# LiZhuoHong/SegLand

Measured on AMD Instinct MI355X. Metric: 512x512 tiles/sec fwd+bwd PSPNet-POP, higher is better.
Workload: dtype bf16; 1 GPU; PSPNet-POP resnet50 bf16, batch 16/GPU, 512x512, 8 logit channels, train_base.py loop body (fwd+loss+bwd+clip+AdamW x2), 1 x MI355X; global_batch=16, parallelism=dp1

## Files before the change

### include/segland_hip_debug.h

```cpp
#ifndef SEGLAND_HIP_DEBUG_H
#define SEGLAND_HIP_DEBUG_H
#include "segland_hip.h"
#ifdef __cplusplus
extern "C" {
#endif

void sl_debug_reset(void);

void sl_debug_conv_affine(int on);
void sl_debug_conv_p9(int on);
void sl_debug_conv_p9_lean(int on);
void sl_debug_conv_p8_k1(int on);
void sl_debug_conv_ring192(int on);
void sl_debug_conv_ringn64(int on);
void sl_debug_conv_rows_small(int on);
void sl_debug_ppm_fact_walk(int on);
void sl_debug_conv_parity(int on);
void sl_debug_ring_small_k(int k);
void sl_debug_ring64_max_tiles(int tiles);
void sl_debug_wgrad3(int on);
void sl_debug_wgrad_bias(int on);
void sl_debug_wgrad_tr(int on);
void sl_debug_wgrad_pair_min(int rows);
void sl_debug_attn_valu(int v);
void sl_debug_ce_tiled(int on);

void sl_debug_p8_trace(void* buf);
void sl_debug_wgrad_trace(void* buf);
void sl_debug_wgrad3_trace(void* buf);
void sl_debug_attn_trace(void* buf);

int sl_debug_wgrad3_plan(const SlConvDesc* d, int* out);

#ifdef __cplusplus
}
#endif
#endif
```

### segland_amd/csrc/api.cpp

```cpp
#include <stdarg.h>
#include <stdio.h>
#include <mutex>
#include <unordered_map>
#include "common.h"

static thread_local char g_err[512] = "";

void sl_set_error(const char* fmt, ...) {
  va_list ap;
  va_start(ap, fmt);
  vsnprintf(g_err, sizeof(g_err), fmt, ap);
  va_end(ap);
}

extern "C" int sl_version(void) { return 100; }
extern "C" const char* sl_last_error_string(void) { return g_err; }

__attribute__((visibility("hidden"))) int sl_lds_opt_in(const char* name, const void* kernel, size_t lds_bytes) {
  static std::mutex mu;
  static std::unordered_map<const void*, size_t> granted;
  std::lock_guard<std::mutex> lock(mu);
  size_t& have = granted[kernel];
  if (lds_bytes <= have) return 0;
  const hipError_t e = hipFuncSetAttribute(kernel, hipFuncAttributeMaxDynamicSharedMemorySize, (int)lds_bytes);
  if (e != hipSuccess) {
    sl_set_error("%s: opt-in to %zu bytes of dynamic LDS refused: %s", name, lds_bytes, hipGetErrorString(e));
    return (int)e;
  }
  have = lds_bytes;
  return 0;
}

extern "C" int sl_hip_clear_error(void) { return (int)hipGetLastError(); }

#include "../../include/segland_hip_debug.h"
SlDebugState g_sl_debug;
extern "C" void sl_debug_reset(void) { g_sl_debug = SlDebugState(); }
extern "C" void sl_debug_conv_affine(int v) { g_sl_debug.conv_affine = v ? 1 : 0; }
extern "C" void sl_debug_conv_p9(int v) { g_sl_debug.conv_p9 = (v & 1) ? 1 : 0; }
extern "C" void sl_debug_conv_p9_lean(int v) { g_sl_debug.conv_p9_lean = v ? 1 : 0; }
extern "C" void sl_debug_conv_p8_k1(int v) { g_sl_debug.conv_p8_k1 = v ? 1 : 0; }
extern "C" void sl_debug_conv_ring192(int v) { g_sl_debug.conv_ring192 = v ? 1 : 0; }
extern "C" void sl_debug_conv_ringn64(int v) { g_sl_debug.conv_ringn64 = v ? 1 : 0; }
extern "C" void sl_debug_conv_rows_small(int v) { g_sl_debug.conv_rows_small = v ? 1 : 0; }
extern "C" void sl_debug_conv_parity(int v) { g_sl_debug.conv_parity = v ? 1 : 0; }
extern "C" void sl_debug_ppm_fact_walk(int v) { g_sl_debug.ppm_fact_walk = v ? 1 : 0; }
extern "C" void sl_debug_ring64_max_tiles(int v) { g_sl_debug.ring64_max_tiles = v; }
extern "C" void sl_debug_ring_small_k(int v) { g_sl_debug.ring_small_k = v; }
extern "C" void sl_debug_wgrad3(int v) { g_sl_debug.wgrad3 = v ? 1 : 0; }
extern "C" void sl_debug_wgrad_bias(int v) { g_sl_debug.wgrad_bias = v ? 1 : 0; }
extern "C" void sl_debug_wgrad_tr(int v) { g_sl_debug.wgrad_tr = v ? 1 : 0; }
extern "C" void sl_debug_wgrad_pair_min(int rows) { g_sl_debug.wgrad_pair_min_rows = rows; }
extern "C" void sl_debug_attn_valu(int v) { g_sl_debug.attn_valu = v; }
extern "C" void sl_debug_ce_tiled(int v) { g_sl_debug.ce_tiled = v ? 1 : 0; }
extern "C" void sl_debug_p8_trace(void* buf) { g_sl_debug.p8_trace = (unsigned long long*)buf; }
extern "C" void sl_debug_wgrad_trace(void* buf) { g_sl_debug.wgrad_trace = (unsigned long long*)buf; }
extern "C" void sl_debug_wgrad3_trace(void* buf) { g_sl_debug.wgrad3_trace = (unsigned long long*)buf; }
extern "C" void sl_debug_attn_trace(void* buf) { g_sl_debug.attn_trace = (unsigned long long*)buf; }
```

### segland_amd/csrc/common.h

```cpp
#pragma once
#include <hip/hip_runtime.h>
#include <stdint.h>
#include <stdio.h>
#include "../../include/segland_hip.h"

typedef unsigned short bf16_t;

typedef __attribute__((ext_vector_type(8))) __bf16 bf16x8_t;
typedef __attribute__((ext_vector_type(16))) float f32x16_t;
typedef __attribute__((ext_vector_type(4))) float f32x4_t;

__device__ __forceinline__ float bf2f(bf16_t v) { return __uint_as_float(((unsigned)v) << 16); }
__device__ __forceinline__ bf16_t f2bf(float f) {
  return __builtin_bit_cast(bf16_t, (__bf16)f);
}

template <typename T> __device__ __forceinline__ float to_f(T v);
template <> __device__ __forceinline__ float to_f<float>(float v) { return v; }
template <> __device__ __forceinline__ float to_f<bf16_t>(bf16_t v) { return bf2f(v); }
template <typename T> __device__ __forceinline__ T from_f(float v);
template <> __device__ __forceinline__ float from_f<float>(float v) { return v; }
template <> __device__ __forceinline__ bf16_t from_f<bf16_t>(float v) { return f2bf(v); }

template <typename T> struct Vec16 { static constexpr int N = 16 / sizeof(T); };
// ... 6 lines not shown
  out[0] = __uint_as_float(v.x << 16); out[1] = __uint_as_float(v.x & 0xffff0000u);
  out[2] = __uint_as_float(v.y << 16); out[3] = __uint_as_float(v.y & 0xffff0000u);
  out[4] = __uint_as_float(v.z << 16); out[5] = __uint_as_float(v.z & 0xffff0000u);
  out[6] = __uint_as_float(v.w << 16); out[7] = __uint_as_float(v.w & 0xffff0000u);
}
template <typename T> __device__ __forceinline__ uint4 pack16(const float* in);
template <> __device__ __forceinline__ uint4 pack16<float>(const float* in) {
  return make_uint4(__float_as_uint(in[0]), __float_as_uint(in[1]), __float_as_uint(in[2]), __float_as_uint(in[3]));
}
template <> __device__ __forceinline__ uint4 pack16<bf16_t>(const float* in) {
  typedef __attribute__((ext_vector_type(2))) __bf16 bf16x2_t;
  typedef __attribute__((ext_vector_type(2))) float f32x2_t;
  uint4 r;
  r.x = __builtin_bit_cast(unsigned, __builtin_convertvector((f32x2_t){in[0], in[1]}, bf16x2_t));
  r.y = __builtin_bit_cast(unsigned, __builtin_convertvector((f32x2_t){in[2], in[3]}, bf16x2_t));
  r.z = __builtin_bit_cast(unsigned, __builtin_convertvector((f32x2_t){in[4], in[5]}, bf16x2_t));
  r.w = __builtin_bit_cast(unsigned, __builtin_convertvector((f32x2_t){in[6], in[7]}, bf16x2_t));
  return r;
}

__device__ __forceinline__ float sl_erf_as(float x) {
  const float ax = fabsf(x);
  const float t = __builtin_amdgcn_rcpf(fmaf(0.3275911f, ax, 1.f));
  float p = fmaf(1.061405429f, t, -1.453152027f);
  p = fmaf(p, t, 1.421413741f); p = fmaf(p, t, -0.284496736f); p = fmaf(p, t, 0.254829592f);
  const float r = fmaf(-p * t, __expf(-ax * ax), 1.f);
  return copysignf(r, x);
}
template <typename T> __device__ __forceinline__ float sl_gelu(float x) {
  if constexpr (sizeof(T) == 4) return 0.5f * x * (1.f + erff(x * 0.70710678118654752440f));
  else return 0.5f * x * (1.f + sl_erf_as(x * 0.70710678118654752440f));
}

template <typename T> __device__ __forceinline__ float sl_gelu_grad(float x) {
  const float pdf = 0.39894228040143267794f * __expf(-0.5f * x * x);
  float cdf;
  if constexpr (sizeof(T) == 4) cdf = 0.5f * (1.f + erff(x * 0.70710678118654752440f));
  else cdf = 0.5f * (1.f + sl_erf_as(x * 0.70710678118654752440f));
  return cdf + x * pdf;
}

__device__ __forceinline__ float wave_sum(float v) {
#pragma unroll
  for (int o = 32; o > 0; o >>= 1) v += __shfl_xor(v, o, 64);
  return v;
}

void sl_set_error(const char* fmt, ...);

struct SlDebugState {
  int conv_affine = 1;
  int conv_p9 = 1;
  int conv_p9_lean = 1;
  int conv_p8_k1 = 1;
  int conv_ring192 = 1;
  int conv_ringn64 = 1;
  int conv_rows_small = 1;
  int ppm_fact_walk = 1;
  int conv_parity = 1;
  int ring_small_k = 128;
  long long ring64_max_tiles = 256;
  int wgrad3 = 1;
  int wgrad_bias = 1;
  int wgrad_tr = 1;
  long long wgrad_pair_min_rows = 0;
  int attn_valu = -1;
  int ce_tiled = 1;
  unsigned long long* p8_trace = nullptr;
  unsigned long long* wgrad_trace = nullptr;
  unsigned long long* wgrad3_trace = nullptr;
  unsigned long long* attn_trace = nullptr;
};
extern SlDebugState g_sl_debug;
#define SL_REQUIRE(cond, ...)            \
  do {                                   \
    if (!(cond)) {                       \
      sl_set_error(__VA_ARGS__);         \
      return SL_EINVAL;                  \
    }                                    \
  } while (0)
#define SL_TRY(expr)                     \
  do {                                   \
    const int rc__ = (expr);             \
    if (rc__) return rc__;               \
  } while (0)

int sl_lds_opt_in(const char* name, const void* kernel, size_t lds_bytes);

template <typename T> struct sl_as_is { typedef T type; };

template <typename... Args>
static inline int sl_launch(const char* name, void (*kernel)(Args...), dim3 grid, dim3 block, size_t lds_bytes, hipStream_t stream, typename sl_as_is<Args>::type... args) {
  if (lds_bytes > 64 * 1024) SL_TRY(sl_lds_opt_in(name, (const void*)kernel, lds_bytes));
  hipLaunchKernelGGL(kernel, grid, block, lds_bytes, stream, args...);
  const hipError_t e = hipGetLastError();
  if (e != hipSuccess) {
    sl_set_error("%s: %s", name, hipGetErrorString(e));
    return (int)e;
  }
  return 0;
}

template <typename F>
static inline int sl_by_dtype(int dtype, const char* entry, F&& f) {
  if (dtype == SL_BF16) return f(bf16_t());
  if (dtype == SL_F32) return f(float());
// ... 62 lines not shown
```

### segland_amd/csrc/conv_gemm.hip

```cpp
#include "conv_gemm_common.h"

using namespace slconv;
namespace {

constexpr int MIN_TILES256 = 96, RING128_MIN = 16;
static int block_rows(long long M) { return M >= 256LL * MIN_TILES256 ? 256 : 128; }

static int splitk_parts(const ConvGemmParams& p, int dtype) {
  if (dtype != SL_BF16 || p.stat_partial || p.gate || p.mask_src || p.addend_mask || p.out2 || p.row_scale || p.C2 || p.N % 256 || p.M % 256 || p.C1 % 64) return 1;
  const long long tiles = (long long)(p.M / 256) * (p.N / 256);
  if (tiles >= 128 || p.M >= 32768 || p.C1 < 1024) return 1;
  if (!(p9_on() && p.KH == 3 && p.KW == 3 && p.stride == 1 && p.pad == p.dil && (p.dil == 1 || p.dil == 2 || p.dil == 4) && p.Hs == p.Hd && p.Ws == p.Wd && p.Hs % 16 == 0 && p.Ws % 16 == 0))
    return 1;
  const int units = p.C1 / 64;
  int s = 1;
  while (s < 8 && units / (2 * s) >= 4 && tiles * 2 * s <= 256) s *= 2;
  return s;
}

static bool ring192_on() { return g_sl_debug.conv_ring192 != 0; }
static bool rows_small_on() { return g_sl_debug.conv_rows_small != 0; }
static bool ringn64_on() { return g_sl_debug.conv_ringn64 != 0; }

static bool parity_shape(const ConvGemmParams& p) {
// ... 107 lines not shown
  SL_REQUIRE(p.M > 0, "conv: empty output");
  SL_REQUIRE(!(p.gate && p.bias), "conv: no kernel serves a gated data gradient with a bias");
  return launch_gemm(dtype, p, st);
}

int check_desc(const SlConvDesc* d) {
  SL_REQUIRE(d != nullptr, "conv: null descriptor");
  SL_REQUIRE(d->B > 0 && d->H > 0 && d->W > 0 && d->Cin > 0 && d->Cout > 0, "conv: bad sizes");
  SL_REQUIRE(d->KH > 0 && d->KW > 0 && d->stride > 0 && d->dil > 0 && d->pad >= 0, "conv: bad window");
  const int ho = (d->H + 2 * d->pad - d->dil * (d->KH - 1) - 1) / d->stride + 1;
  const int wo = (d->W + 2 * d->pad - d->dil * (d->KW - 1) - 1) / d->stride + 1;
  SL_REQUIRE(ho == d->Ho && wo == d->Wo, "conv: Ho/Wo (%d,%d) inconsistent with input (expected %d,%d)", d->Ho, d->Wo, ho, wo);
  SL_REQUIRE(d->C1 > 0 && d->C1 <= d->Cin, "conv: bad C1");
  return 0;
}

}

static ConvGemmParams fwd_params(const SlConvDesc* d) {
  ConvGemmParams p{};
  p.C1 = d->C1; p.C2 = d->Cin - d->C1; p.B = d->B; p.Hs = d->H; p.Ws = d->W; p.Hd = d->Ho; p.Wd = d->Wo; p.N = d->Cout; p.M = d->B * d->Ho * d->Wo;
  p.KH = d->KH; p.KW = d->KW; p.stride = d->stride; p.pad = d->pad; p.dil = d->dil; p.mode = 0;
  return p;
}
static ConvGemmParams dgrad_params(const SlConvDesc* d) {
  ConvGemmParams p{};
  p.C1 = d->Cout; p.C2 = 0; p.B = d->B; p.Hs = d->Ho; p.Ws = d->Wo; p.Hd = d->H; p.Wd = d->W; p.N = d->Cin; p.M = d->B * d->H * d->W;
  p.KH = d->KH; p.KW = d->KW; p.stride = d->stride; p.pad = d->pad; p.dil = d->dil; p.mode = 1;
  return p;
}
static void gated_stats(ConvGemmParams& p, const uint8_t* gate, const void* bn_x, const float* bn_mean, const float* bn_invstd, float* stat_partial) {
  p.gate = gate; p.bn_x = bn_x; p.bn_mean = bn_mean; p.bn_invstd = bn_invstd; p.stat_partial = stat_partial;
}

static unsigned char g_cfg_dummy[16];
static ConvGemmParams query_params(const SlConvDesc* d, int mode, int epi, int addend_half = 0) {
  ConvGemmParams p = mode == 0 ? fwd_params(d) : dgrad_params(d);
  void* dm = (void*)g_cfg_dummy;
  p.src1 = dm; p.wt = dm; p.out = dm;
  if (epi & SL_EPI_STATS) p.stat_partial = (float*)dm;
  if (epi & SL_EPI_AFFINE) { p.scale = (const float*)dm; p.bias = (const float*)dm; p.relu = 1; }
  if (epi & (SL_EPI_ADDEND | SL_EPI_ADDEND_BITS)) p.addend = dm;
  if (epi & SL_EPI_ADDEND_BITS) p.addend_mask = (const unsigned char*)dm;
  if (epi & SL_EPI_GATE) gated_stats(p, (const uint8_t*)dm, dm, (const float*)dm, (const float*)dm, (float*)dm);
  if (epi & SL_EPI_GELU) { p.mask_src = dm; p.flags = 4; }
  p.addend_half = addend_half;
  p.ksplit = (epi & SL_EPI_SPLITK) ? splitk_parts(p, d->dtype) : 1;
  return p;
}
extern "C" int sl_conv2d_tile_config_ex(const SlConvDesc* d, int mode, int epi) {
  if (!d) return SL_EINVAL;
  return choose_kernel(query_params(d, mode, epi), d->dtype).cfg;
}
extern "C" int sl_conv2d_tile_config(const SlConvDesc* d, int mode) { return sl_conv2d_tile_config_ex(d, mode, mode == 0 ? SL_EPI_STATS : 0); }

extern "C" int sl_conv2d_stat_rows(const SlConvDesc* d) {
  if (!d) return SL_EINVAL;
  const ConvGemmParams p = query_params(d, 0, SL_EPI_STATS);
  return (int)stat_rows(choose_kernel(p, d->dtype), p);
}

extern "C" int sl_conv2d_fwd_ex(const SlConvDesc* d, const void* x, const void* x2, const void* w, const void* pre_addend,
                                const float* bias, int relu, void* y, float* stat_partial, sl_stream_t stream) {
  if (int e = check_desc(d)) return e;
  SL_REQUIRE(x && w && y, "conv fwd: null buffer");
  SL_REQUIRE(d->C1 == d->Cin || x2, "conv fwd: x2 missing for a concat input");
  SL_REQUIRE(!(stat_partial && (bias || relu)), "conv fwd: statistics are defined on the raw conv output");
  ConvGemmParams p = fwd_params(d);
  p.src1 = x; p.src2 = x2; p.wt = w; p.out = y;
  p.bias = bias; p.relu = relu; p.stat_partial = stat_partial; p.pre_addend = pre_addend;
  return run_gemm(d->dtype, p, (hipStream_t)stream);
}

extern "C" int sl_conv2d_fwd(const SlConvDesc* d, const void* x, const void* x2, const void* w, const float* bias,
                             int relu, void* y, float* stat_partial, sl_stream_t stream) {
  return sl_conv2d_fwd_ex(d, x, x2, w, nullptr, bias, relu, y, stat_partial, stream);
}

extern "C" int sl_linear_fwd(const SlConvDesc* d, const void* x, const void* w, const float* bias, const float* row_scale, const void* residual,
                             void* y, void* gelu_out, sl_stream_t stream) {
  if (int e = check_desc(d)) return e;
  SL_REQUIRE(x && w && y, "linear fwd: null buffer");
  SL_REQUIRE(d->C1 == d->Cin, "linear fwd: single input tensor");
  ConvGemmParams p = fwd_params(d);
  p.src1 = x; p.wt = w; p.out = y;
  p.bias = bias; p.row_scale = row_scale; p.addend = residual; p.out2 = gelu_out;
  return run_gemm(d->dtype, p, (hipStream_t)stream);
}

extern "C" size_t sl_conv2d_affine_fwd_workspace(const SlConvDesc* d) {
  if (!d || check_desc(d)) return 0;
  const ConvGemmParams p = fwd_params(d);
  const int parts = splitk_parts(p, d->dtype);
  return parts > 1 ? (size_t)parts * p.M * p.N * sizeof(float) : 0;
}

extern "C" int sl_conv2d_affine_fwd_ex(const SlConvDesc* d, const void* x, const void* x2, const void* w, const void* pre_addend, const float* scale,
                                       const float* shift, const void* residual, int relu, void* y, void* workspace, size_t workspace_bytes, sl_stream_t stream) {
  if (int e = check_desc(d)) return e;
  SL_REQUIRE(x && w && y && scale && shift, "conv affine fwd: null buffer");
  SL_REQUIRE(d->C1 == d->Cin || x2, "conv affine fwd: x2 missing for a concat input");
  ConvGemmParams p = fwd_params(d);
  p.src1 = x; p.src2 = x2; p.wt = w; p.out = y;
  p.scale = scale; p.bias = shift; p.relu = relu; p.addend = residual; p.pre_addend = pre_addend;
  const int parts = workspace ? splitk_parts(p, d->dtype) : 1;
  if (parts > 1 && workspace_bytes >= (size_t)parts * p.M * p.N * sizeof(float) && ((size_t)workspace & 15) == 0) { p.ws = (float*)workspace; p.ksplit = parts; }
// ... 93 lines not shown
```

### segland_amd/csrc/conv_gemm_common.h

```cpp
#pragma once
#include <stdlib.h>
#include "common.h"

#ifndef SL_CH3_SPLIT
#define SL_CH3_SPLIT 2
#endif


struct ConvGemmParams {
  const void* src1; const void* src2;
  int C1, C2;
  const void* wt;
  void* out;
  int B, Hs, Ws;
  int Hd, Wd;
  int N, KH, KW, stride, pad, dil;
  int mode;
  const float* scale;
  const float* bias; int relu;
  const void* addend; const void* mask_src;
  const void* pre_addend;
  const unsigned char* addend_mask;
  float* stat_partial;
  const unsigned char* gate;
  const void* bn_x;
  const float* bn_mean; const float* bn_invstd;
  const void* bn_x2; const float* bn_mean2; const float* bn_invstd2; float* stat_partial2;
  int addend_half;
  const float* row_scale;
  void* out2;
  int M;
  int gridM, gridN;
  int tile16;
  int flags;
  float* ws; int ksplit;
  int sub, sub_py, sub_px;
  unsigned long long* trace;
};

namespace slconv __attribute__((visibility("hidden"))) {
constexpr int C64_T = 16;
int launch_tile(int cfg, int dtype, ConvGemmParams& p, hipStream_t st);
int launch_p8(ConvGemmParams& p, hipStream_t st);
int launch_p9(ConvGemmParams& p, hipStream_t st);
bool p9_on();
bool p9_shape(const ConvGemmParams& p);
int launch_c64k3(ConvGemmParams& p, hipStream_t st);
bool c64k3_shape(int dtype, int KH, int KW, int stride, int pad, int dil, int Cin, int C1, int Cout, long long M);
int launch_sk(ConvGemmParams& p, hipStream_t st);
bool sk_shape(int dtype, int KH, int KW, int stride, int pad, int Cin, int C1, int N, long long M);
}

namespace {

template <typename T> struct Mma;
template <> struct Mma<bf16_t> {
  static __device__ __forceinline__ void run(const uint4& a, const uint4& b, f32x16_t& c) {
    c = __builtin_amdgcn_mfma_f32_32x32x16_bf16(__builtin_bit_cast(bf16x8_t, a), __builtin_bit_cast(bf16x8_t, b), c, 0, 0, 0);
  }
};
template <> struct Mma<float> {
  static __device__ __forceinline__ void run(const uint4& a, const uint4& b, f32x16_t& c) {
    c = __builtin_amdgcn_mfma_f32_32x32x2f32(__uint_as_float(a.x), __uint_as_float(b.x), c, 0, 0, 0);
    c = __builtin_amdgcn_mfma_f32_32x32x2f32(__uint_as_float(a.y), __uint_as_float(b.y), c, 0, 0, 0);
    c = __builtin_amdgcn_mfma_f32_32x32x2f32(__uint_as_float(a.z), __uint_as_float(b.z), c, 0, 0, 0);
    c = __builtin_amdgcn_mfma_f32_32x32x2f32(__uint_as_float(a.w), __uint_as_float(b.w), c, 0, 0, 0);
  }
};

__device__ __forceinline__ int lds_off(int row, int chunk) { return row * 128 + ((chunk ^ ((row >> 1) & 7)) << 4); }

template <typename T>
__device__ __forceinline__ void st16(T* dst, const uint4& v) {
  typedef __attribute__((ext_vector_type(4))) unsigned u32x4_t;
  __builtin_nontemporal_store(__builtin_bit_cast(u32x4_t, v), (u32x4_t*)dst);
}

__device__ __forceinline__ void lds_barrier() { asm volatile("s_waitcnt lgkmcnt(0)\n\ts_barrier" ::: "memory"); }

template <typename T, int BM, int BN, int WM, int WN, bool SPLIT = false>
struct EpiGeom {
  static constexpr int PITCH = BN * (int)sizeof(T) + 16;
  static constexpr int TILE_BYTES = BM * PITCH;
  static constexpr int NPASS = (SPLIT || TILE_BYTES > 150 * 1024) ? 2 : 1;
  static constexpr int MAIN_BYTES = 2 * (BM + BN) * 128;
  static constexpr int LDS_BYTES = (TILE_BYTES / NPASS) > MAIN_BYTES ? (TILE_BYTES / NPASS) : MAIN_BYTES;
  static_assert(SPLIT || WM % NPASS == 0, "passes split whole wave rows");
};

template <typename T, int BM, int BN, int WM, int WN, bool SPLIT = false>
__device__ __forceinline__ void epi_stage_acc(f32x16_t (&acc)[BM / WM / 32][BN / WN / 32], int pass, int wm, int wn, int lane, unsigned char* smem) {
  using G = EpiGeom<T, BM, BN, WM, WN, SPLIT>;
  constexpr int TM = BM / WM / 32, TN = BN / WN / 32;
  static_assert(!SPLIT || (G::NPASS == 2 && TM == 4 && TN == 2), "split layout: two passes (operand halves), 4x2 accumulator blocks per wave");
  const int fhalf = lane >> 5;
  if constexpr (!SPLIT) { if (wm / (WM / G::NPASS) != pass) return; }
  const int lrow = SPLIT ? 0 : (wm % (WM / G::NPASS)) * (BM / WM) + (lane & 31);
#pragma unroll
  for (int i = 0; i < TM; ++i)
#pragma unroll
    for (int j = 0; j < TN; ++j)
#pragma unroll
// ... 569 lines not shown
```

### segland_amd/csrc/conv_gemm_sk.hip

```cpp
#include "conv_gemm_common.h"

namespace {

using slconv::C64_T;
constexpr int C64_PW = C64_T + 2, C64_PITCH = 144;
constexpr int C64_WFRAG = 2 * 36 * 64 * 16;
constexpr int C64_LDS = C64_WFRAG + C64_PW * C64_PW * C64_PITCH + 4 * 2 * 64 * (int)sizeof(float);
__global__ __launch_bounds__(256) void conv_c64k3_kernel(ConvGemmParams p, int ntiles) {
  extern __shared__ __attribute__((aligned(16))) unsigned char smem[];
  uint4* wl = (uint4*)smem;
  unsigned char* patch = smem + C64_WFRAG;
  float* red = (float*)(patch + C64_PW * C64_PW * C64_PITCH);
  const int tid = threadIdx.x, lane = tid & 63, wave = tid >> 6, l31 = lane & 31, fh = lane >> 5;
  const int H = p.Hs, W = p.Ws;
  const int tx = cdiv(W, C64_T), ty = cdiv(H, C64_T);
  const bf16_t* src = (const bf16_t*)p.src1;
  for (int e = tid; e < 2 * 36 * 64; e += 256) {
    const int ln = e & 63, ks = (e >> 6) % 36, nb = (e >> 6) / 36;
    wl[e] = *(const uint4*)((const bf16_t*)p.wt + ((size_t)(nb * 32 + (ln & 31)) * 9 + (ks >> 2)) * 64 + (ks & 3) * 16 + (ln >> 5) * 8);
  }
  constexpr int NCH = C64_PW * C64_PW * 8, CPT = (NCH + 255) / 256;
  uint4 stage[CPT];
  auto fetch = [&](int tile) {
    int blk = tile;
    const int bx = blk % tx; blk /= tx;
    const int by = blk % ty; const int b = blk / ty;
#pragma unroll
    for (int u = 0; u < CPT; ++u) {
      const int e = tid + u * 256;
      uint4 v = make_uint4(0, 0, 0, 0);
      if (e < NCH) {
        const int ch8 = e & 7, pp = e >> 3, py = pp / C64_PW, px = pp - py * C64_PW;
        const int iy = by * C64_T - 1 + py, ix = bx * C64_T - 1 + px;
        if ((unsigned)iy < (unsigned)H && (unsigned)ix < (unsigned)W) v = *(const uint4*)(src + ((size_t)(b * H + iy) * W + ix) * 64 + ch8 * 8);
      }
      stage[u] = v;
    }
  };
  int pbase[2];
#pragma unroll
  for (int rb = 0; rb < 2; ++rb) {
    const int pidx = wave * 64 + rb * 32 + l31;
    pbase[rb] = ((pidx >> 4) * C64_PW + (pidx & 15)) * C64_PITCH + fh * 16;
  }
  if ((int)blockIdx.x < ntiles) fetch(blockIdx.x);
  for (int tile = blockIdx.x; tile < ntiles; tile += gridDim.x) {
    int blk = tile;
    const int bx = blk % tx; blk /= tx;
    const int by = blk % ty; const int b = blk / ty;
#pragma unroll
    for (int u = 0; u < CPT; ++u) {
      const int e = tid + u * 256;
// ... 78 lines not shown
          }
        }
      }
    } else
#pragma unroll
    for (int u = 0; u < 8; ++u) {
      const int e = tid + u * 256;
      const int pidx = e >> 3, ch8 = e & 7;
      const int oy = by * C64_T + (pidx >> 4), ox = bx * C64_T + (pidx & 15);
      if (oy < H && ox < W) {
        const uint4 v = *(const uint4*)(outt + pidx * C64_PITCH + ch8 * 16);
        st16(out + ((size_t)(b * H + oy) * W + ox) * 64 + ch8 * 8, v);
        if (p.stat_partial) {
          const unsigned wv[4] = {v.x, v.y, v.z, v.w};
#pragma unroll
          for (int c = 0; c < 4; ++c) {
            const float lo = __uint_as_float(wv[c] << 16), hi = __uint_as_float(wv[c] & 0xffff0000u);
            sa[2 * c] += lo; sq[2 * c] += lo * lo; sa[2 * c + 1] += hi; sq[2 * c + 1] += hi * hi;
          }
        }
      }
    }
    if (p.stat_partial) {
#pragma unroll
      for (int c = 0; c < 8; ++c)
#pragma unroll
        for (int o = 8; o < 64; o <<= 1) { sa[c] += __shfl_xor(sa[c], o); sq[c] += __shfl_xor(sq[c], o); }
      if (lane < 8) {
#pragma unroll
        for (int c = 0; c < 8; ++c) { red[(wave * 2 + 0) * 64 + lane * 8 + c] = sa[c]; red[(wave * 2 + 1) * 64 + lane * 8 + c] = sq[c]; }
      }
      __syncthreads();
      if (tid < 128) {
        const int which = tid >> 6, ch = tid & 63;
        p.stat_partial[((size_t)tile * 2 + which) * 64 + ch] = red[(0 * 2 + which) * 64 + ch] + red[(1 * 2 + which) * 64 + ch] + red[(2 * 2 + which) * 64 + ch] + red[(3 * 2 + which) * 64 + ch];
      }
    }
    __syncthreads();
  }
}

}

bool slconv::c64k3_shape(int dtype, int KH, int KW, int stride, int pad, int dil, int Cin, int C1, int Cout, long long M) {
  return dtype == SL_BF16 && KH == 3 && KW == 3 && stride == 1 && pad == 1 && dil == 1 && Cin == 64 && C1 == 64 && Cout == 64 && M >= 65536;
}

int slconv::launch_c64k3(ConvGemmParams& p, hipStream_t st) {
  const int ntiles = p.B * cdiv(p.Hs, C64_T) * cdiv(p.Ws, C64_T);
  return sl_launch("conv_c64k3_kernel", conv_c64k3_kernel, dim3(ntiles < 256 ? ntiles : 256), dim3(256), C64_LDS, st, p, ntiles);
}

namespace {
template <int KS> struct SkGeom {
  static constexpr int RB = KS * 32;
  static constexpr int BSTEP = 64 * RB;
  static constexpr int STG_PITCH = 144, STG_WAVE = 32 * STG_PITCH;
  static constexpr int OFF_STG = 2 * BSTEP, OFF_RED = OFF_STG + 8 * STG_WAVE;
  static constexpr int LDS = OFF_RED + 2 * 8 * 3 * 64 * (int)sizeof(float);
};
template <int KS> __device__ __forceinline__ int sk_swz(int row) { return KS == 16 ? (row & 31) : (KS == 8 ? (row & 15) : ((row >> 1) & 7)); }
__device__ __forceinline__ float sk_sum_8_16_32(float v) {
  typedef __attribute__((ext_vector_type(2))) unsigned u32x2_t;
  v += __int_as_float(__builtin_amdgcn_update_dpp(0, __float_as_int(v), 0x128, 0xf, 0xf, false));
  u32x2_t r = __builtin_amdgcn_permlane16_swap(__float_as_uint(v), __float_as_uint(v), false, false);
  v = __uint_as_float(r.x) + __uint_as_float(r.y);
  r = __builtin_amdgcn_permlane32_swap(__float_as_uint(v), __float_as_uint(v), false, false);
  return __uint_as_float(r.x) + __uint_as_float(r.y);
}

#ifndef SL_SK_ABL
#define SL_SK_ABL 0
#endif
template <int KS, int MODE, bool SKEW>
__global__ __launch_bounds__(512, (KS == 4 && MODE != 5) ? 4 : 2) void conv_gemm_sk_kernel(ConvGemmParams p) {
  using G = SkGeom<KS>;
  using T = bf16_t;
  typedef __attribute__((ext_vector_type(2))) __bf16 bf16x2_t;
  typedef __attribute__((ext_vector_type(2))) float f32x2_t;
  extern __shared__ __attribute__((aligned(16))) unsigned char smem[];
  const int tid = threadIdx.x, lane = tid & 63;
  const int wave = __builtin_amdgcn_readfirstlane(tid >> 6);
  const int grp = wave >> 2;
  const int l31 = lane & 31, fh = lane >> 5;
  const int bm = blockIdx.x;
  const int NS = p.N / 64;
  const unsigned lds_base = __builtin_amdgcn_readfirstlane(lds_addr_of(smem));
  constexpr int NWI = SKEW ? 4 : 8, NI = 2 * KS / NWI, LPR = 2 * KS, RPI = 64 / LPR;
  const int iw = SKEW ? (wave & 3) : wave;
  const bool issuer = !SKEW || grp == 0;
  const unsigned char* bsrc[NI];
#pragma unroll
  for (int j = 0; j < NI; ++j) {
    const int row = (iw * NI + j) * RPI + lane / LPR, pos = lane % LPR;
    bsrc[j] = (const unsigned char*)p.wt + (size_t)row * G::RB + ((pos ^ sk_swz<KS>(row)) << 4);
  }
  auto issueB = [&](int s, int buf) {
#pragma unroll
    for (int j = 0; j < NI; ++j) glds16_asm(bsrc[j] + (size_t)s * G::BSTEP, lds_base + buf * G::BSTEP + (iw * NI + j) * 1024);
  };
  auto colstep = [&](int i) { return i; };
  if (issuer) issueB(colstep(0), 0);
  uint4 a[KS];
  {
    const unsigned char* arow = (const unsigned char*)p.src1 + ((size_t)bm * 256 + wave * 32 + l31) * G::RB + fh * 16;
#pragma unroll
    for (int ks = 0; ks < KS; ++ks) a[ks] = *(const uint4*)(arow + ks * 32);
  }
  int foff[KS];
  {
    const int x = sk_swz<KS>(l31);
#pragma unroll
    for (int ks = 0; ks < KS; ++ks) foff[ks] = l31 * G::RB + (((2 * ks + fh) ^ x) << 4);
  }
  unsigned char* stg = smem + G::OFF_STG + wave * G::STG_WAVE;
  float* red = (float*)(smem + G::OFF_RED);
  const int srow = lane >> 3, sch = lane & 7;
  const size_t orow = (size_t)bm * 256 + wave * 32 + srow;
  long long arow[4];
  if constexpr (MODE == 2 || MODE == 5) {
#pragma unroll
    for (int it = 0; it < 4; ++it) {
      const long long m = (long long)orow + it * 8;
      arow[it] = m;
      if (p.addend_half) {
        const int hw = p.Hd * p.Wd;
        const int b = (int)(m / hw), rem = (int)(m - (long long)b * hw), y = rem / p.Wd, x = rem - y * p.Wd;
        arow[it] = ((y | x) & 1) ? -1 : ((long long)b * (p.Hd >> 1) + (y >> 1)) * (p.Wd >> 1) + (x >> 1);
      }
    }
  }
  uint4 addv[4], cxv[4], cxv2[4];
  float bmu[8], bis[8], bmu2[8], bis2[8];
  const bool dual = MODE == 5 && p.bn_x2 != nullptr;
  const int mpitch = p.N / 8 + 16;
  unsigned char* msk = smem + (MODE == 5 ? G::LDS : G::OFF_RED);
  if ((MODE == 2 && p.addend_mask) || MODE == 5) {
    const int cpr = p.N / 128;
    const unsigned char* src = (MODE == 5 ? p.gate : p.addend_mask) + (size_t)bm * 256 * (p.N / 8);
    for (int e = tid; e < 256 * cpr; e += 512) {
      const int row = e / cpr, c = e - row * cpr;
      *(uint4*)(msk + row * mpitch + c * 16) = *(const uint4*)(src + (size_t)e * 16);
    }
  }

  auto multiply = [&](int i) {
    const int cur = i & 1, s = colstep(i);
    if (issuer && i + 1 < NS) issueB(colstep(i + 1), cur ^ 1);
    if constexpr (MODE == 2 || MODE == 5) {
      const int ncol = s * 64 + sch * 8;
#pragma unroll
      for (int it = 0; it < 4; ++it) addv[it] = (arow[it] >= 0 && !(SL_SK_ABL & 2)) ? *(const uint4*)((const T*)p.addend + arow[it] * p.N + ncol) : make_uint4(0, 0, 0, 0);
      if constexpr (MODE == 5) {
#pragma unroll
        for (int it = 0; it < 4; ++it) cxv[it] = (SL_SK_ABL & 2) ? make_uint4(0, 0, 0, 0) : *(const uint4*)((const T*)p.bn_x + (orow + it * 8) * p.N + ncol);
#pragma unroll
        for (int e = 0; e < 8; ++e) { bmu[e] = p.bn_mean[ncol + e]; bis[e] = p.bn_invstd[ncol + e]; }
        if (dual) {
#pragma unroll
          for (int it = 0; it < 4; ++it) cxv2[it] = *(const uint4*)((const T*)p.bn_x2 + (orow + it * 8) * p.N + ncol);
#pragma unroll
          for (int e = 0; e < 8; ++e) { bmu2[e] = p.bn_mean2[ncol + e]; bis2[e] = p.bn_invstd2[ncol + e]; }
        }
      }
    }
    f32x16_t acc[2];
#pragma unroll
    for (int j = 0; j < 2; ++j)
#pragma unroll
      for (int r = 0; r < 16; ++r) acc[j][r] = 0.f;
    const unsigned char* bb = smem + cur * G::BSTEP;
#pragma unroll
    for (int ks = 0; ks < KS; ++ks) {
      const uint4 b0 = *(const uint4*)(bb + foff[ks]), b1 = *(const uint4*)(bb + 32 * G::RB + foff[ks]);
      if constexpr (!(SL_SK_ABL & 8)) {
      Mma<T>::run(b0, a[ks], acc[0]);
      Mma<T>::run(b1, a[ks], acc[1]);
      } else { acc[0][0] += __uint_as_float(b0.x); acc[1][0] += __uint_as_float(b1.x); }
    }
#pragma unroll
    for (int j = 0; j < 2; ++j)
#pragma unroll
      for (int q = 0; q < 4; ++q) {
        uint2 v;
        v.x = __builtin_bit_cast(unsigned, __builtin_convertvector((f32x2_t){acc[j][4 * q + 0], acc[j][4 * q + 1]}, bf16x2_t));
        v.y = __builtin_bit_cast(unsigned, __builtin_convertvector((f32x2_t){acc[j][4 * q + 2], acc[j][4 * q + 3]}, bf16x2_t));
        *(uint2*)(stg + l31 * G::STG_PITCH + 64 * j + 16 * q + 8 * fh) = v;
      }
  };

  auto store = [&](int i) {
    const int cur = i & 1, s = colstep(i);
    const int ncol = s * 64 + sch * 8;
    wait_vmcnt<0>();
    float sa[8], sq[8], sq2[8];
#pragma unroll
    for (int e = 0; e < 8; ++e) { sa[e] = 0.f; sq[e] = 0.f; sq2[e] = 0.f; }
#pragma unroll
    for (int it = 0; it < 4; ++it) {
      const uint4 raw = *(const uint4*)(stg + (it * 8 + srow) * G::STG_PITCH + sch * 16);
      T* o = (T*)p.out + (orow + it * 8) * p.N + ncol;
      if constexpr (MODE == 1) {
        st16(o, raw);
        if (p.stat_partial) {
          const unsigned w[4] = {raw.x, raw.y, raw.z, raw.w};
#pragma unroll
          for (int c = 0; c < 4; ++c) {
            const float lo = __uint_as_float(w[c] << 16), hi = __uint_as_float(w[c] & 0xffff0000u);
            sa[2 * c] += lo; sq[2 * c] += lo * lo; sa[2 * c + 1] += hi; sq[2 * c + 1] += hi * hi;
          }
        }
      } else {
        uint4 ad = addv[it];
        if (MODE == 2 && p.addend_mask) {
          const unsigned b = msk[(wave * 32 + it * 8 + srow) * mpitch + s * 8 + sch];
          ad.x &= ((unsigned)__builtin_amdgcn_sbfe(b, 0, 1) & 0xffffu) | ((unsigned)__builtin_amdgcn_sbfe(b, 1, 1) & 0xffff0000u);
          ad.y &= ((unsigned)__builtin_amdgcn_sbfe(b, 2, 1) & 0xffffu) | ((unsigned)__builtin_amdgcn_sbfe(b, 3, 1) & 0xffff0000u);
          ad.z &= ((unsigned)__builtin_amdgcn_sbfe(b, 4, 1) & 0xffffu) | ((unsigned)__builtin_amdgcn_sbfe(b, 5, 1) & 0xffff0000u);
          ad.w &= ((unsigned)__builtin_amdgcn_sbfe(b, 6, 1) & 0xffffu) | ((unsigned)__builtin_amdgcn_sbfe(b, 7, 1) & 0xffff0000u);
        }
        const unsigned rw[4] = {raw.x, raw.y, raw.z, raw.w}, aw[4] = {ad.x, ad.y, ad.z, ad.w};
        unsigned ow[4];
#pragma unroll
        for (int c = 0; c < 4; ++c) {
          const f32x2_t v = (f32x2_t){__uint_as_float(rw[c] << 16) + __uint_as_float(aw[c] << 16), __uint_as_float(rw[c] & 0xffff0000u) + __uint_as_float(aw[c] & 0xffff0000u)};
          ow[c] = __builtin_bit_cast(unsigned, __builtin_convertvector(v, bf16x2_t));
        }
        if constexpr (MODE == 5) {
          const unsigned b = msk[(wave * 32 + it * 8 + srow) * mpitch + s * 8 + sch];
          ow[0] &= ((unsigned)__builtin_amdgcn_sbfe(b, 0, 1) & 0xffffu) | ((unsigned)__builtin_amdgcn_sbfe(b, 1, 1) & 0xffff0000u);
          ow[1] &= ((unsigned)__builtin_amdgcn_sbfe(b, 2, 1) & 0xffffu) | ((unsigned)__builtin_amdgcn_sbfe(b, 3, 1) & 0xffff0000u);
          ow[2] &= ((unsigned)__builtin_amdgcn_sbfe(b, 4, 1) & 0xffffu) | ((unsigned)__builtin_amdgcn_sbfe(b, 5, 1) & 0xffff0000u);
          ow[3] &= ((unsigned)__builtin_amdgcn_sbfe(b, 6, 1) & 0xffffu) | ((unsigned)__builtin_amdgcn_sbfe(b, 7, 1) & 0xffff0000u);
          const unsigned xw[4] = {cxv[it].x, cxv[it].y, cxv[it].z, cxv[it].w};
#pragma unroll
          for (int c = 0; c < 4; ++c) {
            if constexpr (SL_SK_ABL & 4) { sa[2 * c] += __uint_as_float(ow[c] ^ xw[c]); continue; }
            const float glo = __uint_as_float(ow[c] << 16), ghi = __uint_as_float(ow[c] & 0xffff0000u);
            const float xlo = __uint_as_float(xw[c] << 16), xhi = __uint_as_float(xw[c] & 0xffff0000u);
            sa[2 * c] += glo; sq[2 * c] += glo * ((xlo - bmu[2 * c]) * bis[2 * c]);
            sa[2 * c + 1] += ghi; sq[2 * c + 1] += ghi * ((xhi - bmu[2 * c + 1]) * bis[2 * c + 1]);
          }
          if (dual) {
            const unsigned yw[4] = {cxv2[it].x, cxv2[it].y, cxv2[it].z, cxv2[it].w};
#pragma unroll
            for (int c = 0; c < 4; ++c) {
              const float glo = __uint_as_float(ow[c] << 16), ghi = __uint_as_float(ow[c] & 0xffff0000u);
              const float ylo = __uint_as_float(yw[c] << 16), yhi = __uint_as_float(yw[c] & 0xffff0000u);
              sq2[2 * c] += glo * ((ylo - bmu2[2 * c]) * bis2[2 * c]);
              sq2[2 * c + 1] += ghi * ((yhi - bmu2[2 * c + 1]) * bis2[2 * c + 1]);
            }
          }
        }
        if constexpr (SL_SK_ABL & 1) { if (ow[0] == 0x12345678u && ow[1] == 0x9abcdef0u) st16(o, make_uint4(ow[0], ow[1], ow[2], ow[3])); }
        else st16(o, make_uint4(ow[0], ow[1], ow[2], ow[3]));
      }
    }
    if ((MODE == 1 || MODE == 5) && p.stat_partial) {
#pragma unroll
      for (int e = 0; e < 8; ++e) { sa[e] = sk_sum_8_16_32(sa[e]); sq[e] = sk_sum_8_16_32(sq[e]); }
      if (dual) {
#pragma unroll
        for (int e = 0; e < 8; ++e) sq2[e] = sk_sum_8_16_32(sq2[e]);
      }
      if (lane < 8) {
        float* r0 = red + ((cur * 8 + wave) * 3) * 64 + sch * 8;
        *(float4*)(r0) = make_float4(sa[0], sa[1], sa[2], sa[3]); *(float4*)(r0 + 4) = make_float4(sa[4], sa[5], sa[6], sa[7]);
        *(float4*)(r0 + 64) = make_float4(sq[0], sq[1], sq[2], sq[3]); *(float4*)(r0 + 68) = make_float4(sq[4], sq[5], sq[6], sq[7]);
        if (dual) { *(float4*)(r0 + 128) = make_float4(sq2[0], sq2[1], sq2[2], sq2[3]); *(float4*)(r0 + 132) = make_float4(sq2[4], sq2[5], sq2[6], sq2[7]); }
      }
    }
  };
  auto finalize = [&](int i, int t0) {
    const int s = colstep(i);
    if ((MODE == 1 || MODE == 5) && p.stat_partial && tid >= t0 && tid < t0 + (dual ? 192 : 128)) {
      const int which = (tid - t0) >> 6, col = tid & 63;
      const float* r0 = red + ((i & 1) * 24 + which) * 64 + col;
      float t = 0.f;
#pragma unroll
      for (int k = 0; k < 8; ++k) t += r0[k * 192];
      if (which < 2) p.stat_partial[((size_t)bm * 2 + which) * p.N + s * 64 + col] = t;
      if (dual && which != 1) p.stat_partial2[((size_t)bm * 2 + (which >> 1)) * p.N + s * 64 + col] = t;
    }
  };

  auto bar = [&]() { asm volatile("s_waitcnt lgkmcnt(0)\n\ts_barrier" ::: "memory"); };
  wait_vmcnt<0>();
  bar();
  if constexpr (!SKEW) {
#pragma unroll 1
    for (int s = 0; s < NS; ++s) {
      multiply(s);
      store(s);
      bar();
      finalize(s, 0);
    }
  } else if (grp == 0) {
#pragma unroll 1
    for (int s = 0; s < NS; ++s) {
      multiply(s);
      bar();
      store(s);
      bar();
    }
    bar();
  } else {
    bar();
#pragma unroll 1
    for (int s = 0; s < NS; ++s) {
      multiply(s);
      bar();
      store(s);
      bar();
      finalize(s, 256);
    }
  }
}

}

bool slconv::sk_shape(int dtype, int KH, int KW, int stride, int pad, int Cin, int C1, int N, long long M) {
  return dtype == SL_BF16 && KH == 1 && KW == 1 && stride == 1 && pad == 0 && C1 == Cin && (Cin == 64 || Cin == 128 || Cin == 256) &&
         N % 64 == 0 && M >= 65536 && M % 256 == 0;
}

namespace {
template <int KS, int MODE, bool SKEW>
int launch_sk_t(ConvGemmParams& p, hipStream_t st) {
  const int lds = MODE == 5 ? SkGeom<KS>::LDS + 256 * (p.N / 8 + 16)
                            : (MODE == 2 && p.addend_mask ? SkGeom<KS>::OFF_RED + 256 * (p.N / 8 + 16) : SkGeom<KS>::LDS);
  return sl_launch("conv_gemm_sk_kernel", conv_gemm_sk_kernel<KS, MODE, SKEW>, dim3(p.M / 256), dim3(512), lds, st, p);
}
template <int MODE, bool SKEW>
int launch_sk_k(ConvGemmParams& p, hipStream_t st) {
  return p.C1 == 256 ? launch_sk_t<16, MODE, SKEW>(p, st) : (p.C1 == 128 ? launch_sk_t<8, MODE, SKEW>(p, st) : launch_sk_t<4, MODE, SKEW>(p, st));
}
}

int slconv::launch_sk(ConvGemmParams& p, hipStream_t st) {
  constexpr int skew = 1;
  p.gridM = p.M / 256; p.gridN = 1;
  if (p.gate) return launch_sk_k<5, false>(p, st);
  if (p.addend) return (skew & 4) ? launch_sk_k<2, true>(p, st) : launch_sk_k<2, false>(p, st);
  return (skew & (p.stat_partial ? 1 : 2)) ? launch_sk_k<1, true>(p, st) : launch_sk_k<1, false>(p, st);
}
```

Before: 726.3 tiles/s.

## Add pipelined multi-slot schedule to 1x1 sk conv GEMM kernel

Adds a PIPE variant of the sk 1x1 conv GEMM kernel. It prefetches B tiles one or two steps ahead into two or three LDS slots and double-buffers the addend and bn_x epilogue loads in registers, using inline-asm loads and partial vmcnt waits. The variant is chosen by default for small grids (at most 2x the CU count) in specific addend and gate cases, with the number of slots picked by an LDS budget. It trades more LDS and registers (occupancy drops to 2 waves/SIMD for KS=4) for overlapping global loads with MFMA and epilogue work.

```diff
diff --git a/include/segland_hip_debug.h b/include/segland_hip_debug.h
--- a/include/segland_hip_debug.h
+++ b/include/segland_hip_debug.h
@@ -11,6 +11,7 @@
 void sl_debug_conv_p9(int on);
 void sl_debug_conv_p9_lean(int on);
 void sl_debug_conv_p8_k1(int on);
+void sl_debug_conv_sk_pipe(int on);
 void sl_debug_conv_ring192(int on);
 void sl_debug_conv_ringn64(int on);
 void sl_debug_conv_rows_small(int on);
@@ -30,6 +31,8 @@
 void sl_debug_wgrad3_trace(void* buf);
 void sl_debug_attn_trace(void* buf);
 
+int sl_debug_conv_sk_pipe_slots(const SlConvDesc* d, int mode, int epi, int addend_half);
+
 int sl_debug_wgrad3_plan(const SlConvDesc* d, int* out);
 
 #ifdef __cplusplus
diff --git a/segland_amd/csrc/api.cpp b/segland_amd/csrc/api.cpp
--- a/segland_amd/csrc/api.cpp
+++ b/segland_amd/csrc/api.cpp
@@ -39,6 +39,7 @@
 extern "C" void sl_debug_conv_affine(int v) { g_sl_debug.conv_affine = v ? 1 : 0; }
 extern "C" void sl_debug_conv_p9(int v) { g_sl_debug.conv_p9 = (v & 1) ? 1 : 0; }
 extern "C" void sl_debug_conv_p9_lean(int v) { g_sl_debug.conv_p9_lean = v ? 1 : 0; }
+extern "C" void sl_debug_conv_sk_pipe(int v) { g_sl_debug.conv_sk_pipe = v == 0 ? 0 : (v == 1 ? 1 : 2); }
 extern "C" void sl_debug_conv_p8_k1(int v) { g_sl_debug.conv_p8_k1 = v ? 1 : 0; }
 extern "C" void sl_debug_conv_ring192(int v) { g_sl_debug.conv_ring192 = v ? 1 : 0; }
 extern "C" void sl_debug_conv_ringn64(int v) { g_sl_debug.conv_ringn64 = v ? 1 : 0; }
diff --git a/segland_amd/csrc/common.h b/segland_amd/csrc/common.h
--- a/segland_amd/csrc/common.h
+++ b/segland_amd/csrc/common.h
@@ -82,6 +82,7 @@
   int conv_affine = 1;
   int conv_p9 = 1;
   int conv_p9_lean = 1;
+  int conv_sk_pipe = 1;
   int conv_p8_k1 = 1;
   int conv_ring192 = 1;
   int conv_ringn64 = 1;
diff --git a/segland_amd/csrc/conv_gemm.hip b/segland_amd/csrc/conv_gemm.hip
--- a/segland_amd/csrc/conv_gemm.hip
+++ b/segland_amd/csrc/conv_gemm.hip
@@ -183,6 +183,11 @@
   if (!d) return SL_EINVAL;
   return choose_kernel(query_params(d, mode, epi), d->dtype).cfg;
 }
+extern "C" int sl_debug_conv_sk_pipe_slots(const SlConvDesc* d, int mode, int epi, int addend_half) {
+  if (!d) return 0;
+  const ConvGemmParams p = query_params(d, mode, epi, addend_half);
+  return choose_kernel(p, d->dtype).cfg == 6256064 ? sk_pipe_slots(p) : 0;
+}
 extern "C" int sl_conv2d_tile_config(const SlConvDesc* d, int mode) { return sl_conv2d_tile_config_ex(d, mode, mode == 0 ? SL_EPI_STATS : 0); }
 
 extern "C" int sl_conv2d_stat_rows(const SlConvDesc* d) {
diff --git a/segland_amd/csrc/conv_gemm_common.h b/segland_amd/csrc/conv_gemm_common.h
--- a/segland_amd/csrc/conv_gemm_common.h
+++ b/segland_amd/csrc/conv_gemm_common.h
@@ -48,6 +48,7 @@
 int launch_c64k3(ConvGemmParams& p, hipStream_t st);
 bool c64k3_shape(int dtype, int KH, int KW, int stride, int pad, int dil, int Cin, int C1, int Cout, long long M);
 int launch_sk(ConvGemmParams& p, hipStream_t st);
+int sk_pipe_slots(const ConvGemmParams& p);
 bool sk_shape(int dtype, int KH, int KW, int stride, int pad, int Cin, int C1, int N, long long M);
 }
 
diff --git a/segland_amd/csrc/conv_gemm_sk.hip b/segland_amd/csrc/conv_gemm_sk.hip
--- a/segland_amd/csrc/conv_gemm_sk.hip
+++ b/segland_amd/csrc/conv_gemm_sk.hip
@@ -1,3 +1,4 @@
+#include <type_traits>
 #include "conv_gemm_common.h"
 
 namespace {
@@ -182,11 +183,11 @@
 }
 
 namespace {
-template <int KS> struct SkGeom {
+template <int KS, int SLOTS = 2> struct SkGeom {
   static constexpr int RB = KS * 32;
   static constexpr int BSTEP = 64 * RB;
   static constexpr int STG_PITCH = 144, STG_WAVE = 32 * STG_PITCH;
-  static constexpr int OFF_STG = 2 * BSTEP, OFF_RED = OFF_STG + 8 * STG_WAVE;
+  static constexpr int OFF_STG = SLOTS * BSTEP, OFF_RED = OFF_STG + 8 * STG_WAVE;
   static constexpr int LDS = OFF_RED + 2 * 8 * 3 * 64 * (int)sizeof(float);
 };
 template <int KS> __device__ __forceinline__ int sk_swz(int row) { return KS == 16 ? (row & 31) : (KS == 8 ? (row & 15) : ((row >> 1) & 7)); }
@@ -202,9 +203,14 @@
 #ifndef SL_SK_ABL
 #define SL_SK_ABL 0
 #endif
-template <int KS, int MODE, bool SKEW>
-__global__ __launch_bounds__(512, (KS == 4 && MODE != 5) ? 4 : 2) void conv_gemm_sk_kernel(ConvGemmParams p) {
-  using G = SkGeom<KS>;
+typedef __attribute__((ext_vector_type(4))) unsigned sk_u32x4_t;
+__device__ __forceinline__ void sk_gld16_sbase_asm(sk_u32x4_t& d, const void* sbase, unsigned voff) { asm volatile("global_load_dwordx4 %0, %1, %2" : "=&v"(d) : "v"(voff), "s"(sbase) : "memory"); }
+__device__ __forceinline__ void sk_pin(sk_u32x4_t (&v)[4]) { asm volatile("" : "+v"(v[0]), "+v"(v[1]), "+v"(v[2]), "+v"(v[3]) : : "memory"); }
+
+template <int KS, int MODE, bool SKEW, int PIPE = 0>
+__global__ __launch_bounds__(512, (KS == 4 && MODE != 5 && !PIPE) ? 4 : 2) void conv_gemm_sk_kernel(ConvGemmParams p) {
+  static_assert(!(PIPE && SKEW) && (PIPE == 0 || PIPE == 2 || PIPE == 3) && (!PIPE || MODE != 5 || KS < 16), "the pipelined schedule is un-skewed, on two or three slots; its MODE 5 fits the registers up to K = 128");
+  using G = SkGeom<KS, PIPE ? PIPE : 2>;
   using T = bf16_t;
   typedef __attribute__((ext_vector_type(2))) __bf16 bf16x2_t;
   typedef __attribute__((ext_vector_type(2))) float f32x2_t;
@@ -262,7 +268,7 @@
   }
   uint4 addv[4], cxv[4], cxv2[4];
   float bmu[8], bis[8], bmu2[8], bis2[8];
-  const bool dual = MODE == 5 && p.bn_x2 != nullptr;
+  const bool dual = !PIPE && MODE == 5 && p.bn_x2 != nullptr;
   const int mpitch = p.N / 8 + 16;
   unsigned char* msk = smem + (MODE == 5 ? G::LDS : G::OFF_RED);
   if ((MODE == 2 && p.addend_mask) || MODE == 5) {
@@ -274,6 +280,32 @@
     }
   }
 
+  auto mma = [&](int cur) {
+    f32x16_t acc[2];
+#pragma unroll
+    for (int j = 0; j < 2; ++j)
+#pragma unroll
+      for (int r = 0; r < 16; ++r) acc[j][r] = 0.f;
+    const unsigned char* bb = smem + cur * G::BSTEP;
+#pragma unroll
+    for (int ks = 0; ks < KS; ++ks) {
+      const int fo = PIPE ? (foff[0] ^ (ks << 5)) : foff[ks];
+      const uint4 b0 = *(const uint4*)(bb + fo), b1 = *(const uint4*)(bb + 32 * G::RB + fo);
+      if constexpr (!(SL_SK_ABL & 8)) {
+      Mma<T>::run(b0, a[ks], acc[0]);
+      Mma<T>::run(b1, a[ks], acc[1]);
+      } else { acc[0][0] += __uint_as_float(b0.x); acc[1][0] += __uint_as_float(b1.x); }
+    }
+#pragma unroll
+    for (int j = 0; j < 2; ++j)
+#pragma unroll
+      for (int q = 0; q < 4; ++q) {
+        uint2 v;
+        v.x = __builtin_bit_cast(unsigned, __builtin_convertvector((f32x2_t){acc[j][4 * q + 0], acc[j][4 * q + 1]}, bf16x2_t));
+        v.y = __builtin_bit_cast(unsigned, __builtin_convertvector((f32x2_t){acc[j][4 * q + 2], acc[j][4 * q + 3]}, bf16x2_t));
+        *(uint2*)(stg + l31 * G::STG_PITCH + 64 * j + 16 * q + 8 * fh) = v;
+      }
+  };
   auto multiply = [&](int i) {
     const int cur = i & 1, s = colstep(i);
     if (issuer && i + 1 < NS) issueB(colstep(i + 1), cur ^ 1);
@@ -294,35 +326,13 @@
         }
       }
     }
-    f32x16_t acc[2];
-#pragma unroll
-    for (int j = 0; j < 2; ++j)
-#pragma unroll
-      for (int r = 0; r < 16; ++r) acc[j][r] = 0.f;
-    const unsigned char* bb = smem + cur * G::BSTEP;
-#pragma unroll
-    for (int ks = 0; ks < KS; ++ks) {
-      const uint4 b0 = *(const uint4*)(bb + foff[ks]), b1 = *(const uint4*)(bb + 32 * G::RB + foff[ks]);
-      if constexpr (!(SL_SK_ABL & 8)) {
-      Mma<T>::run(b0, a[ks], acc[0]);
-      Mma<T>::run(b1, a[ks], acc[1]);
-      } else { acc[0][0] += __uint_as_float(b0.x); acc[1][0] += __uint_as_float(b1.x); }
-    }
-#pragma unroll
-    for (int j = 0; j < 2; ++j)
-#pragma unroll
-      for (int q = 0; q < 4; ++q) {
-        uint2 v;
-        v.x = __builtin_bit_cast(unsigned, __builtin_convertvector((f32x2_t){acc[j][4 * q + 0], acc[j][4 * q + 1]}, bf16x2_t));
-        v.y = __builtin_bit_cast(unsigned, __builtin_convertvector((f32x2_t){acc[j][4 * q + 2], acc[j][4 * q + 3]}, bf16x2_t));
-        *(uint2*)(stg + l31 * G::STG_PITCH + 64 * j + 16 * q + 8 * fh) = v;
-      }
-  };
-
-  auto store = [&](int i) {
+    mma(cur);
+  };
+
+  auto store_core = [&](int i, const uint4 (&addv)[4], const uint4 (&cxv)[4], const uint4 (&cxv2)[4], const float (&bmu)[8], const float (&bis)[8], const float (&bmu2)[8],
+                        const float (&bis2)[8]) {
     const int cur = i & 1, s = colstep(i);
     const int ncol = s * 64 + sch * 8;
-    wait_vmcnt<0>();
     float sa[8], sq[8], sq2[8];
 #pragma unroll
     for (int e = 0; e < 8; ++e) { sa[e] = 0.f; sq[e] = 0.f; sq2[e] = 0.f; }
@@ -401,6 +411,10 @@
       }
     }
   };
+  auto store = [&](int i) {
+    wait_vmcnt<0>();
+    store_core(i, addv, cxv, cxv2, bmu, bis, bmu2, bis2);
+  };
   auto finalize = [&](int i, int t0) {
     const int s = colstep(i);
     if ((MODE == 1 || MODE == 5) && p.stat_partial && tid >= t0 && tid < t0 + (dual ? 192 : 128)) {
@@ -415,6 +429,92 @@
   };
 
   auto bar = [&]() { asm volatile("s_waitcnt lgkmcnt(0)\n\ts_barrier" ::: "memory"); };
+  if constexpr (PIPE != 0) {
+    constexpr int FA = PIPE - 1;
+    constexpr int SC = (SL_SK_ABL & 1) ? 0 : 4;
+    constexpr bool LD = (MODE == 2 || MODE == 5) && !(SL_SK_ABL & 2);
+    constexpr int NL = !LD ? 0 : (MODE == 2 ? 4 : 8);
+    using c0_t = std::integral_constant<int, 0>;
+    using c1_t = std::integral_constant<int, 1>;
+    unsigned aoff[4], avalid = 0;
+    const unsigned boff = (unsigned)(((wave * 32 + srow) * p.N + sch * 8) * (int)sizeof(T));
+    const size_t brow = (size_t)8 * p.N * sizeof(T), bblk = (size_t)bm * 256 * p.N * sizeof(T);
+    sk_u32x4_t la[2][4], lc[2][4];
+    if constexpr (MODE == 2 || MODE == 5) {
+#pragma unroll
+      for (int it = 0; it < 4; ++it) {
+        aoff[it] = (unsigned)(((size_t)(arow[it] < 0 ? 0 : arow[it]) * p.N + sch * 8) * sizeof(T));
+        avalid |= (arow[it] >= 0 ? 1u : 0u) << it;
+#pragma unroll
+        for (int q = 0; q < 2; ++q) { la[q][it] = (sk_u32x4_t){0, 0, 0, 0}; lc[q][it] = (sk_u32x4_t){0, 0, 0, 0}; }
+      }
+    }
+    auto issueL = [&](auto P, int s) {
+      constexpr int Pv = decltype(P)::value;
+      if constexpr (LD) {
+        const size_t c = (size_t)s * (64 * sizeof(T));
+#pragma unroll
+        for (int it = 0; it < 4; ++it) sk_gld16_sbase_asm(la[Pv][it], (const unsigned char*)p.addend + c, aoff[it]);
+        if constexpr (MODE == 5) {
+#pragma unroll
+          for (int it = 0; it < 4; ++it) sk_gld16_sbase_asm(lc[Pv][it], (const unsigned char*)p.bn_x + bblk + it * brow + c, boff);
+        }
+      }
+    };
+    const float* bnl = (const float*)(msk + 256 * mpitch);
+    if constexpr (MODE == 5) {
+      float* w = (float*)(msk + 256 * mpitch);
+      for (int e = tid; e < p.N; e += 512) { w[e] = p.bn_mean[e]; w[p.N + e] = p.bn_invstd[e]; }
+    }
+    if (FA == 2 && NS > 1) issueB(1, 1);
+    issueL(c0_t(), 0);
+    wait_vmcnt<0>();
+    bar();
+    auto step = [&](auto P, int i, int slot) {
+      constexpr int Pv = decltype(P)::value;
+      const bool hasF = i + FA < NS, hasL = i + 1 < NS;
+      if (FA == 1 && hasF) issueB(i + 1, slot ^ 1);
+      mma(slot);
+      if (FA == 2 && hasF) issueB(i + 2, slot == 0 ? 2 : slot - 1);
+      if (hasL) issueL(std::integral_constant<int, Pv ^ 1>(), i + 1);
+      if (hasF) wait_vmcnt<SC + NI + NL>();
+      else if (hasL) wait_vmcnt<SC + NL>();
+      else wait_vmcnt<SC>();
+      uint4 ad[4], cx[4];
+      float mu[8], is[8];
+      if constexpr (MODE == 2 || MODE == 5) {
+        sk_pin(la[Pv]);
+#pragma unroll
+        for (int it = 0; it < 4; ++it) ad[it] = ((avalid >> it) & 1) ? __builtin_bit_cast(uint4, la[Pv][it]) : make_uint4(0, 0, 0, 0);
+      }
+      if constexpr (MODE == 5) {
+        sk_pin(lc[Pv]);
+        const float* bc = bnl + i * 64 + sch * 8;
+#pragma unroll
+        for (int it = 0; it < 4; ++it) cx[it] = __builtin_bit_cast(uint4, lc[Pv][it]);
+#pragma unroll
+        for (int h = 0; h < 2; ++h) {
+          const float4 m4 = *(const float4*)(bc + 4 * h), s4 = *(const float4*)(bc + p.N + 4 * h);
+          mu[4 * h] = m4.x; mu[4 * h + 1] = m4.y; mu[4 * h + 2] = m4.z; mu[4 * h + 3] = m4.w;
+          is[4 * h] = s4.x; is[4 * h + 1] = s4.y; is[4 * h + 2] = s4.z; is[4 * h + 3] = s4.w;
+        }
+      }
+      store_core(i, ad, cx, cxv2, mu, is, bmu2, bis2);
+      if (FA == 1 && hasF) wait_vmcnt<SC + NL>();
+      bar();
+      finalize(i, 0);
+    };
+    int slot = 0, i = 0;
+#pragma unroll 1
+    for (; i + 1 < NS; i += 2) {
+      step(c0_t(), i, slot);
+      slot = slot + 1 == PIPE ? 0 : slot + 1;
+      step(c1_t(), i + 1, slot);
+      slot = slot + 1 == PIPE ? 0 : slot + 1;
+    }
+    if (i < NS) step(c0_t(), i, slot);
+    return;
+  }
   wait_vmcnt<0>();
   bar();
   if constexpr (!SKEW) {
@@ -455,21 +555,42 @@
 }
 
 namespace {
-template <int KS, int MODE, bool SKEW>
+constexpr int SK_LDS_MAX = 160 * 1024, SK_CUS = 256;
+static int sk_lds_bytes(const ConvGemmParams& p, int slots, bool pipe) {
+  const int bstep = 64 * p.C1 * 2, off_red = slots * bstep + 8 * 32 * 144, full = off_red + 2 * 8 * 3 * 64 * (int)sizeof(float), bits = 256 * (p.N / 8 + 16);
+  if (p.gate) return full + bits + (pipe ? 2 * p.N * (int)sizeof(float) : 0);
+  return p.addend && p.addend_mask ? off_red + bits : full;
+}
+template <int KS, int MODE, bool SKEW, int PIPE = 0>
 int launch_sk_t(ConvGemmParams& p, hipStream_t st) {
-  const int lds = MODE == 5 ? SkGeom<KS>::LDS + 256 * (p.N / 8 + 16)
-                            : (MODE == 2 && p.addend_mask ? SkGeom<KS>::OFF_RED + 256 * (p.N / 8 + 16) : SkGeom<KS>::LDS);
-  return sl_launch("conv_gemm_sk_kernel", conv_gemm_sk_kernel<KS, MODE, SKEW>, dim3(p.M / 256), dim3(512), lds, st, p);
-}
-template <int MODE, bool SKEW>
+  static_assert(SkGeom<KS, 3>::LDS == SkGeom<KS>::LDS + SkGeom<KS>::BSTEP && SkGeom<KS>::BSTEP == 64 * KS * 16 * 2 && SkGeom<KS>::STG_WAVE == 32 * 144, "sk_lds_bytes mirrors SkGeom");
+  return sl_launch("conv_gemm_sk_kernel", conv_gemm_sk_kernel<KS, MODE, SKEW, PIPE>, dim3(p.M / 256), dim3(512), sk_lds_bytes(p, PIPE ? PIPE : 2, PIPE != 0), st, p);
+}
+template <int MODE, bool SKEW, int PIPE = 0>
 int launch_sk_k(ConvGemmParams& p, hipStream_t st) {
-  return p.C1 == 256 ? launch_sk_t<16, MODE, SKEW>(p, st) : (p.C1 == 128 ? launch_sk_t<8, MODE, SKEW>(p, st) : launch_sk_t<4, MODE, SKEW>(p, st));
-}
+  if constexpr (PIPE && MODE == 5) return p.C1 == 128 ? launch_sk_t<8, MODE, SKEW, PIPE>(p, st) : launch_sk_t<4, MODE, SKEW, PIPE>(p, st);
+  else return p.C1 == 256 ? launch_sk_t<16, MODE, SKEW, PIPE>(p, st) : (p.C1 == 128 ? launch_sk_t<8, MODE, SKEW, PIPE>(p, st) : launch_sk_t<4, MODE, SKEW, PIPE>(p, st));
+}
+template <int MODE>
+int launch_sk_pipe(ConvGemmParams& p, hipStream_t st, int slots) { return slots == 3 ? launch_sk_k<MODE, false, 3>(p, st) : launch_sk_k<MODE, false, 2>(p, st); }
+}
+
+int slconv::sk_pipe_slots(const ConvGemmParams& p) {
+  constexpr int kinds[3] = {0, 4 | 8, 4};
+  const int kind = p.gate ? 8 : (p.addend ? 4 : (p.stat_partial ? 1 : 2)), k = p.C1 == 256 ? 2 : (p.C1 == 128 ? 1 : 0);
+  if (!g_sl_debug.conv_sk_pipe || (long long)p.M * p.N * 2 >= (1LL << 32)) return 0;
+  if (p.gate && (p.bn_x2 || p.C1 == 256)) return 0;
+  if (g_sl_debug.conv_sk_pipe == 1 && (p.M / 256 > 2 * SK_CUS || !(kinds[k] & kind))) return 0;
+  return sk_lds_bytes(p, 3, true) <= SK_LDS_MAX ? 3 : 2;
 }
 
 int slconv::launch_sk(ConvGemmParams& p, hipStream_t st) {
   constexpr int skew = 1;
   p.gridM = p.M / 256; p.gridN = 1;
+  if (const int slots = sk_pipe_slots(p)) {
+    if (p.gate) return launch_sk_pipe<5>(p, st, slots);
+    return p.addend ? launch_sk_pipe<2>(p, st, slots) : launch_sk_pipe<1>(p, st, slots);
+  }
   if (p.gate) return launch_sk_k<5, false>(p, st);
   if (p.addend) return (skew & 4) ? launch_sk_k<2, true>(p, st) : launch_sk_k<2, false>(p, st);
   return (skew & (p.stat_partial ? 1 : 2)) ? launch_sk_k<1, true>(p, st) : launch_sk_k<1, false>(p, st);
```

Result: no change. 728.7 tiles/s, median of 6 (+0.3%).
